# bdsaglam/torch-scae

Measured on AMD Instinct MI355X. Metric: images/sec SCAE fwd+bwd, MNIST 40x40 bs=128, 1/2/4/8 MI355X, higher is better.
Workload: dtype f32

## Files before the change

### torch_scae_amd/csrc/conv_resident.hip

```cpp
#include <cstdlib>

#include "bf16x6.h"
#include "mfma_pipe.h"
#include "conv_first_dev.h"

namespace {
namespace pipe = scae_pipe;
using scae_first::ConvGeom;
constexpr int NT = 256;

struct ResArgs {
  const float *in, *wp, *bias, *post_bias;
  float *out, *out_post;
  ConvGeom g;
  int G;
};

template <int MI>
__global__ __launch_bounds__(NT, 2) void conv_res_fwd_kernel(ResArgs a) {
  constexpr bool X6 = true;
  extern __shared__ __attribute__((aligned(1024))) float smem[];
  const int tid = threadIdx.x, wid = __builtin_amdgcn_readfirstlane(tid >> 6), lane = tid & 63,
            li = lane & 31, lk = lane >> 5;
  const ConvGeom &g = a.g;
  const int ntiles = g.Cout / 32;
  const int nt = blockIdx.x % ntiles, img0 = (blockIdx.x / ntiles) * a.G;
  const int nimg = min(a.G, g.B - img0);
  const int ipix = g.IH * g.IW, opix = g.OH * g.OW;
  const int SP = g.Cin / 4;
  {
    const pipe::rsrc_t rin =
        pipe::make_rsrc(a.in, (unsigned)((size_t)g.B * ipix * g.Cin * 4));
    const int units = a.G * ipix * SP, pieces = (units + 63) / 64;
    const int valid = nimg * ipix;
    for (int j = wid; j < pieces; j += 4) {
      const int u = j * 64 + lane, p = u / SP, s = u - p * SP;
      const int vo = p < valid ? (((img0 * ipix + p) * g.Cin) + ((s ^ (p & 15)) << 2)) * 4
                               : pipe::DMA_ZERO;
      pipe::dma16(rin, smem + j * 256, vo, 0);
    }
  }
  const int rows = nimg * opix;
  int pbase[MI];
#pragma unroll
  for (int mi = 0; mi < MI; ++mi) {
    const int r = min(mi * 32 + li, rows - 1);
    const int n = r / opix, rem = r - n * opix, oh = rem / g.OW, ow = rem - oh * g.OW;
    pbase[mi] = n * ipix + oh * g.stride * g.IW + ow * g.stride;
  }
  const int CB = g.Cin / 32;
  const int CPT = CB / 4;
  const int NCW = 9 * CPT;
  const uint4 *wq = reinterpret_cast<const uint4 *>(a.wp) + (size_t)nt * (9 * CB) * 384 + lane;
  constexpr int NS = !X6 ? 1 : (MI == 1 ? 3 : 1);
  pipe::f32x16 acc[MI], accl[X6 ? MI : 1][NS];
#pragma unroll
  for (int mi = 0; mi < MI; ++mi)
#pragma unroll
    for (int e = 0; e < 16; ++e) {
      acc[mi][e] = 0.f;
      if (X6) {
#pragma unroll
        for (int n = 0; n < NS; ++n) accl[mi][n][e] = 0.f;
      }
    }
  uint4 bq[2][2][3];
  auto load_b = [&](int c, int buf) {
    const int tap = c / CPT, cb = wid + 4 * (c - tap * CPT);
    const uint4 *src = wq + (size_t)(tap * CB + cb) * 384;
#pragma unroll
    for (int qp = 0; qp < 2; ++qp)
#pragma unroll
      for (int pl = 0; pl < 3; ++pl) bq[buf][qp][pl] = src[(qp * 3 + pl) * 64];
  };
  load_b(0, 0);
  pipe::wait_vm<0>();
  __syncthreads();
  auto chunk = [&](int c, int buf) {
    if (c + 1 < NCW) load_b(c + 1, buf ^ 1);
    const int tap = c / CPT, cb = wid + 4 * (c - tap * CPT);
    const int kh = tap / 3, kw = tap - 3 * kh;
    const int slot0 = cb * 8 + lk * 4;
    const float *ap[MI];
    int sw[MI];
#pragma unroll
    for (int mi = 0; mi < MI; ++mi) {
      const int p = pbase[mi] + kh * g.IW + kw;
      ap[mi] = smem + p * g.Cin;
      sw[mi] = p & 15;
    }
    if (X6) {
#pragma unroll
      for (int qp = 0; qp < 2; ++qp) {
        scae_x6::Split3 bs;
        bs.hi = __builtin_bit_cast(scae_x6::bf16x8, bq[buf][qp][0]);
        bs.mid = __builtin_bit_cast(scae_x6::bf16x8, bq[buf][qp][1]);
        bs.lo = __builtin_bit_cast(scae_x6::bf16x8, bq[buf][qp][2]);
        scae_x6::Split3 as[MI];
#pragma unroll
        for (int mi = 0; mi < MI; ++mi) {
          const float4 a0 = pipe::lds4(ap[mi] + (((slot0 + 2 * qp) ^ sw[mi]) << 2));
          const float4 a1 = pipe::lds4(ap[mi] + (((slot0 + 2 * qp + 1) ^ sw[mi]) << 2));
          as[mi] = scae_x6::split3(a0, a1);
        }
#define SCAE_X6_STEP(AP, BP, N)                                                                   \
  _Pragma("unroll") for (int mi = 0; mi < MI; ++mi) accl[mi][(N) % NS] =                          \
      __builtin_amdgcn_mfma_f32_32x32x16_bf16(as[mi].AP, bs.BP, accl[mi][(N) % NS], 0, 0, 0);
        SCAE_X6_STEP(hi, lo, 0)
        SCAE_X6_STEP(lo, hi, 1)
        SCAE_X6_STEP(mid, mid, 2)
        SCAE_X6_STEP(hi, mid, 0)
        SCAE_X6_STEP(mid, hi, 1)
#undef SCAE_X6_STEP
#pragma unroll
        for (int mi = 0; mi < MI; ++mi)
          acc[mi] = __builtin_amdgcn_mfma_f32_32x32x16_bf16(as[mi].hi, bs.hi, acc[mi], 0, 0, 0);
      }
    }
  };
  for (int c = 0; c < NCW; c += 2) {
    chunk(c, 0);
    if (c + 1 < NCW) chunk(c + 1, 1);
  }
  if (X6) {
#pragma unroll
    for (int mi = 0; mi < MI; ++mi) {
      pipe::f32x16 small = accl[mi][0];
#pragma unroll
      for (int n = 1; n < NS; ++n) small += accl[mi][n];
      acc[mi] += small;
    }
  }
  __syncthreads();
#pragma unroll
  for (int mi = 0; mi < MI; ++mi)
#pragma unroll
    for (int e = 0; e < 16; ++e) smem[((wid * MI + mi) * 16 + e) * 64 + lane] = acc[mi][e];
  const int col = nt * 32 + li;
  const float bn = a.bias[col];
  float pb[MI][4];
  const int row0 = 8 * wid + 4 * lk;
  if (a.out_post) {
#pragma unroll
    for (int mi = 0; mi < MI; ++mi)
#pragma unroll
      for (int e = 0; e < 4; ++e) {
        const int r = min(mi * 32 + row0 + e, rows - 1);
        pb[mi][e] = a.post_bias[(size_t)col * opix + r % opix];
      }
  }
  __syncthreads();
  const unsigned obytes = (unsigned)((size_t)g.B * opix * g.Cout * 4);
  const pipe::rsrc_t ro = pipe::make_rsrc(a.out, obytes);
  const pipe::rsrc_t rp = pipe::make_rsrc(a.out_post ? a.out_post : a.out, obytes);
#pragma unroll
  for (int mi = 0; mi < MI; ++mi)
#pragma unroll
    for (int e = 0; e < 4; ++e) {
      float v = 0.f;
#pragma unroll
      for (int w = 0; w < 4; ++w) v += smem[((w * MI + mi) * 16 + 4 * wid + e) * 64 + lane];
      const int r = mi * 32 + row0 + e;
      const float o = fmaxf(v + bn, 0.f);
      const int off = r < rows ? ((img0 * opix + r) * g.Cout + col) * 4 : pipe::DMA_ZERO;
      __builtin_amdgcn_raw_buffer_store_b32(__builtin_bit_cast(int, o), ro, off, 0, 0);
      if (a.out_post)
        __builtin_amdgcn_raw_buffer_store_b32(__builtin_bit_cast(int, o + pb[mi][e]), rp, off, 0, 0);
    }
}

struct ResPlan {
  int G, MI;
  size_t lds;
};
bool res_plan(const ConvGeom &g, ResPlan &p, int force_g) {
  if (g.stride < 1 || g.stride > 2 || g.Cin % 128 || g.Cout % 32) return false;
  const int opix = g.OH * g.OW, ipix = g.IH * g.IW;
  double best = 0.;
  p.G = 0;
  for (int G = 1; G <= 8 && G <= g.B; ++G) {
    if (force_g > 0 && G != force_g) continue;
    const int MI = (G * opix + 31) / 32;
    const size_t stage = ((size_t)G * ipix * g.Cin * 4 + 1023) & ~(size_t)1023;
    const size_t lds = std::max(stage, (size_t)4 * MI * 16 * 64 * 4);
    if (MI > 4 || lds > (force_g > 0 ? 150 : 64) * 1024) break;
    const double use = (double)G * opix / (32. * MI);
    if (use > best + 1e-9) best = use, p.G = G, p.MI = MI, p.lds = lds;
  }
  return p.G > 0;
}
}

extern "C" int scae_conv3x3_fwd_res_supported(int B, int IH, int IW, int Cin, int Cout, int stride) {
  if (B <= 0 || IH < 3 || IW < 3 || Cin <= 0 || Cout <= 0 || stride <= 0) return 0;
  ConvGeom g{B, IH, IW, (IH - 3) / stride + 1, (IW - 3) / stride + 1, Cin, Cout, stride};
  ResPlan p;
  return res_plan(g, p, 0) ? 1 : 0;
}

extern "C" int scae_conv3x3_fwd_res_f32(const float *in, const float *wp, const float *bias,
                                        float *out, const float *post_bias, float *out_post, int B,
                                        int IH, int IW, int Cin, int Cout, int stride, int group,
                                        void *stream) {
  SCAE_REQUIRE(in && wp && bias && out && (!out_post || post_bias) && B > 0 && IH >= 3 && IW >= 3 &&
               Cin > 0 && Cout > 0 && stride > 0 && group >= 0);
  ConvGeom g{B, IH, IW, (IH - 3) / stride + 1, (IW - 3) / stride + 1, Cin, Cout, stride};
  ResPlan p;
  if (!res_plan(g, p, group)) return SCAE_ERR_UNSUPPORTED;
  ResArgs a{in, wp, bias, post_bias, out, out_post, g, p.G};
  const dim3 grid((Cout / 32) * ((B + p.G - 1) / p.G));
  hipStream_t st = (hipStream_t)stream;
#define SCAE_RES(M)                                                                              \
  case M: {                                                                                      \
    if (p.lds > 48 * 1024) {                                                                     \
      hipError_t e = hipFuncSetAttribute(reinterpret_cast<const void *>(conv_res_fwd_kernel<M>), \
                                         hipFuncAttributeMaxDynamicSharedMemorySize, (int)p.lds); \
      if (e != hipSuccess) return (int)e;                                                        \
    }                                                                                            \
    scae::launch(conv_res_fwd_kernel<M>, grid, dim3(NT), p.lds, st, a);                          \
    break;                                                                                       \
  }
  switch (p.MI) {
    SCAE_RES(1) SCAE_RES(2) SCAE_RES(3) SCAE_RES(4)
    default: return SCAE_ERR_UNSUPPORTED;
  }
#undef SCAE_RES
  return scae_launch_status();
}
```

Baseline: 269,500.

## Pre-split staged conv input into bf16x3 in LDS and share across two N tiles

The resident 3x3 conv kernel now splits each fp32 input into hi/mid/lo bf16 parts once, while staging it into LDS, using a 48-byte unit layout with an output-pixel-keyed swizzle. Before, every wave re-split the same activations for every tap and column tile. Blocks can also run 512 threads covering two 32-column output tiles, so one staged image is reused by twice as many columns. The LDS budget rises to 80KB and staging now goes through registers instead of direct DMA. In exchange, the small float-based division and the halved occupancy bound for NJ=2 could reduce latency hiding.

Result: faster. 273,600, median of 6 (+1.5%).

```diff
diff --git a/torch_scae_amd/csrc/conv_resident.hip b/torch_scae_amd/csrc/conv_resident.hip
--- a/torch_scae_amd/csrc/conv_resident.hip
+++ b/torch_scae_amd/csrc/conv_resident.hip
@@ -16,120 +16,149 @@
   int G;
 };
 
-template <int MI>
-__global__ __launch_bounds__(NT, 2) void conv_res_fwd_kernel(ResArgs a) {
-  constexpr bool X6 = true;
+constexpr int SU = 6;
+constexpr int UNIT_BYTES = 48;
+
+__device__ __forceinline__ int small_div(int p, float rd) { return (int)(((float)p + 0.5f) * rd); }
+
+template <int MI, int NJ>
+__global__ __launch_bounds__(NT * NJ, 2 / NJ) void conv_res_fwd_kernel(ResArgs a) {
+  constexpr int NTH = NT * NJ;
   extern __shared__ __attribute__((aligned(1024))) float smem[];
+  char *const simg = reinterpret_cast<char *>(smem);
   const int tid = threadIdx.x, wid = __builtin_amdgcn_readfirstlane(tid >> 6), lane = tid & 63,
             li = lane & 31, lk = lane >> 5;
   const ConvGeom &g = a.g;
-  const int ntiles = g.Cout / 32;
-  const int nt = blockIdx.x % ntiles, img0 = (blockIdx.x / ntiles) * a.G;
+  const int kp = wid & 3, nj = wid >> 2;
+  const int ntiles = g.Cout / (32 * NJ);
+  const int nt = (blockIdx.x % ntiles) * NJ + nj, img0 = (blockIdx.x / ntiles) * a.G;
   const int nimg = min(a.G, g.B - img0);
   const int ipix = g.IH * g.IW, opix = g.OH * g.OW;
-  const int SP = g.Cin / 4;
+  const int UP = g.Cin / 8;
+  const int rowb = UP * UNIT_BYTES;
+  const int sh = g.stride - 1;
+  const int CB = g.Cin / 32;
+  const int CPT = CB / 4;
+  const int NCW = 9 * CPT;
+  const uint4 *wq = reinterpret_cast<const uint4 *>(a.wp) + (size_t)nt * (9 * CB) * 384 + lane;
+  uint4 bq[2][2][3];
+  auto load_b = [&](int c, int buf) {
+    const int tap = c / CPT, cb = kp + 4 * (c - tap * CPT);
+    const uint4 *src = wq + (size_t)(tap * CB + cb) * 384;
+#pragma unroll
+    for (int qp = 0; qp < 2; ++qp)
+#pragma unroll
+      for (int pl = 0; pl < 3; ++pl) bq[buf][qp][pl] = src[(qp * 3 + pl) * 64];
+  };
+  load_b(0, 0);
   {
     const pipe::rsrc_t rin =
         pipe::make_rsrc(a.in, (unsigned)((size_t)g.B * ipix * g.Cin * 4));
-    const int units = a.G * ipix * SP, pieces = (units + 63) / 64;
-    const int valid = nimg * ipix;
-    for (int j = wid; j < pieces; j += 4) {
-      const int u = j * 64 + lane, p = u / SP, s = u - p * SP;
-      const int vo = p < valid ? (((img0 * ipix + p) * g.Cin) + ((s ^ (p & 15)) << 2)) * 4
-                               : pipe::DMA_ZERO;
-      pipe::dma16(rin, smem + j * 256, vo, 0);
+    const int units = a.G * ipix * UP, valid = nimg * ipix;
+    const float ripix = 1.f / (float)ipix, riw = 1.f / (float)g.IW;
+    const int dp = NTH / UP, ds = NTH - dp * UP;
+    int p = tid / UP, s = tid - p * UP;
+    for (int ub = 0; ub < units; ub += SU * NTH) {
+      const int u0 = ub + tid;
+      scae_x6::u32x4 v[SU][2];
+      int dst[SU];
+#pragma unroll
+      for (int k = 0; k < SU; ++k) {
+        if (ub + k * NTH >= units) break;
+        const bool in = u0 + k * NTH < units;
+        const int vo = in && p < valid ? ((img0 * ipix + p) * g.Cin + s * 8) * 4 : pipe::DMA_ZERO;
+        v[k][0] = __builtin_amdgcn_raw_buffer_load_b128(rin, vo, 0, 0);
+        v[k][1] = __builtin_amdgcn_raw_buffer_load_b128(rin, vo, 16, 0);
+        const int n = small_div(p, ripix), rem = p - n * ipix;
+        const int ih = small_div(rem, riw), iw = rem - ih * g.IW;
+        const int key = n * opix + (ih >> sh) * g.OW + (iw >> sh);
+        dst[k] = in ? p * rowb + (s ^ (key & 15)) * UNIT_BYTES : units * UNIT_BYTES;
+        s += ds, p += dp;
+        if (s >= UP) s -= UP, ++p;
+      }
+#pragma unroll
+      for (int k = 0; k < SU; ++k) {
+        if (ub + k * NTH >= units) break;
+        const scae_x6::Split3 sp = scae_x6::split3(__builtin_bit_cast(float4, v[k][0]),
+                                                   __builtin_bit_cast(float4, v[k][1]));
+        uint4 *d = reinterpret_cast<uint4 *>(simg + dst[k]);
+        d[0] = __builtin_bit_cast(uint4, sp.hi);
+        d[1] = __builtin_bit_cast(uint4, sp.mid);
+        d[2] = __builtin_bit_cast(uint4, sp.lo);
+      }
     }
   }
   const int rows = nimg * opix;
-  int pbase[MI];
+  int pbase[MI], kbase[MI];
 #pragma unroll
   for (int mi = 0; mi < MI; ++mi) {
     const int r = min(mi * 32 + li, rows - 1);
     const int n = r / opix, rem = r - n * opix, oh = rem / g.OW, ow = rem - oh * g.OW;
     pbase[mi] = n * ipix + oh * g.stride * g.IW + ow * g.stride;
-  }
-  const int CB = g.Cin / 32;
-  const int CPT = CB / 4;
-  const int NCW = 9 * CPT;
-  const uint4 *wq = reinterpret_cast<const uint4 *>(a.wp) + (size_t)nt * (9 * CB) * 384 + lane;
-  constexpr int NS = !X6 ? 1 : (MI == 1 ? 3 : 1);
-  pipe::f32x16 acc[MI], accl[X6 ? MI : 1][NS];
+    kbase[mi] = r;
+  }
+  constexpr int NS = MI == 1 ? 3 : 1;
+  pipe::f32x16 acc[MI], accl[MI][NS];
 #pragma unroll
   for (int mi = 0; mi < MI; ++mi)
 #pragma unroll
     for (int e = 0; e < 16; ++e) {
       acc[mi][e] = 0.f;
-      if (X6) {
-#pragma unroll
-        for (int n = 0; n < NS; ++n) accl[mi][n][e] = 0.f;
-      }
-    }
-  uint4 bq[2][2][3];
-  auto load_b = [&](int c, int buf) {
-    const int tap = c / CPT, cb = wid + 4 * (c - tap * CPT);
-    const uint4 *src = wq + (size_t)(tap * CB + cb) * 384;
-#pragma unroll
-    for (int qp = 0; qp < 2; ++qp)
-#pragma unroll
-      for (int pl = 0; pl < 3; ++pl) bq[buf][qp][pl] = src[(qp * 3 + pl) * 64];
-  };
-  load_b(0, 0);
-  pipe::wait_vm<0>();
+#pragma unroll
+      for (int n = 0; n < NS; ++n) accl[mi][n][e] = 0.f;
+    }
   __syncthreads();
   auto chunk = [&](int c, int buf) {
     if (c + 1 < NCW) load_b(c + 1, buf ^ 1);
-    const int tap = c / CPT, cb = wid + 4 * (c - tap * CPT);
+    const int tap = c / CPT, cb = kp + 4 * (c - tap * CPT);
     const int kh = tap / 3, kw = tap - 3 * kh;
-    const int slot0 = cb * 8 + lk * 4;
-    const float *ap[MI];
+    const int unit0 = cb * 4 + lk * 2;
+    const char *ap[MI];
     int sw[MI];
 #pragma unroll
     for (int mi = 0; mi < MI; ++mi) {
-      const int p = pbase[mi] + kh * g.IW + kw;
-      ap[mi] = smem + p * g.Cin;
-      sw[mi] = p & 15;
-    }
-    if (X6) {
-#pragma unroll
-      for (int qp = 0; qp < 2; ++qp) {
-        scae_x6::Split3 bs;
-        bs.hi = __builtin_bit_cast(scae_x6::bf16x8, bq[buf][qp][0]);
-        bs.mid = __builtin_bit_cast(scae_x6::bf16x8, bq[buf][qp][1]);
-        bs.lo = __builtin_bit_cast(scae_x6::bf16x8, bq[buf][qp][2]);
-        scae_x6::Split3 as[MI];
-#pragma unroll
-        for (int mi = 0; mi < MI; ++mi) {
-          const float4 a0 = pipe::lds4(ap[mi] + (((slot0 + 2 * qp) ^ sw[mi]) << 2));
-          const float4 a1 = pipe::lds4(ap[mi] + (((slot0 + 2 * qp + 1) ^ sw[mi]) << 2));
-          as[mi] = scae_x6::split3(a0, a1);
-        }
+      ap[mi] = simg + (pbase[mi] + kh * g.IW + kw) * rowb;
+      sw[mi] = (kbase[mi] + (kh >> sh) * g.OW + (kw >> sh)) & 15;
+    }
+#pragma unroll
+    for (int qp = 0; qp < 2; ++qp) {
+      scae_x6::Split3 bs;
+      bs.hi = __builtin_bit_cast(scae_x6::bf16x8, bq[buf][qp][0]);
+      bs.mid = __builtin_bit_cast(scae_x6::bf16x8, bq[buf][qp][1]);
+      bs.lo = __builtin_bit_cast(scae_x6::bf16x8, bq[buf][qp][2]);
+      scae_x6::Split3 as[MI];
+#pragma unroll
+      for (int mi = 0; mi < MI; ++mi) {
+        const uint4 *src =
+            reinterpret_cast<const uint4 *>(ap[mi] + ((unit0 + qp) ^ sw[mi]) * UNIT_BYTES);
+        as[mi].hi = __builtin_bit_cast(scae_x6::bf16x8, src[0]);
+        as[mi].mid = __builtin_bit_cast(scae_x6::bf16x8, src[1]);
+        as[mi].lo = __builtin_bit_cast(scae_x6::bf16x8, src[2]);
+      }
 #define SCAE_X6_STEP(AP, BP, N)                                                                   \
   _Pragma("unroll") for (int mi = 0; mi < MI; ++mi) accl[mi][(N) % NS] =                          \
       __builtin_amdgcn_mfma_f32_32x32x16_bf16(as[mi].AP, bs.BP, accl[mi][(N) % NS], 0, 0, 0);
-        SCAE_X6_STEP(hi, lo, 0)
-        SCAE_X6_STEP(lo, hi, 1)
-        SCAE_X6_STEP(mid, mid, 2)
-        SCAE_X6_STEP(hi, mid, 0)
-        SCAE_X6_STEP(mid, hi, 1)
+      SCAE_X6_STEP(hi, lo, 0)
+      SCAE_X6_STEP(lo, hi, 1)
+      SCAE_X6_STEP(mid, mid, 2)
+      SCAE_X6_STEP(hi, mid, 0)
+      SCAE_X6_STEP(mid, hi, 1)
 #undef SCAE_X6_STEP
 #pragma unroll
-        for (int mi = 0; mi < MI; ++mi)
-          acc[mi] = __builtin_amdgcn_mfma_f32_32x32x16_bf16(as[mi].hi, bs.hi, acc[mi], 0, 0, 0);
-      }
+      for (int mi = 0; mi < MI; ++mi)
+        acc[mi] = __builtin_amdgcn_mfma_f32_32x32x16_bf16(as[mi].hi, bs.hi, acc[mi], 0, 0, 0);
     }
   };
   for (int c = 0; c < NCW; c += 2) {
     chunk(c, 0);
     if (c + 1 < NCW) chunk(c + 1, 1);
   }
-  if (X6) {
-#pragma unroll
-    for (int mi = 0; mi < MI; ++mi) {
-      pipe::f32x16 small = accl[mi][0];
-#pragma unroll
-      for (int n = 1; n < NS; ++n) small += accl[mi][n];
-      acc[mi] += small;
-    }
+#pragma unroll
+  for (int mi = 0; mi < MI; ++mi) {
+    pipe::f32x16 small = accl[mi][0];
+#pragma unroll
+    for (int n = 1; n < NS; ++n) small += accl[mi][n];
+    acc[mi] += small;
   }
   __syncthreads();
 #pragma unroll
@@ -139,7 +168,7 @@
   const int col = nt * 32 + li;
   const float bn = a.bias[col];
   float pb[MI][4];
-  const int row0 = 8 * wid + 4 * lk;
+  const int row0 = 8 * kp + 4 * lk;
   if (a.out_post) {
 #pragma unroll
     for (int mi = 0; mi < MI; ++mi)
@@ -159,7 +188,8 @@
     for (int e = 0; e < 4; ++e) {
       float v = 0.f;
 #pragma unroll
-      for (int w = 0; w < 4; ++w) v += smem[((w * MI + mi) * 16 + 4 * wid + e) * 64 + lane];
+      for (int w = 0; w < 4; ++w)
+        v += smem[(((nj * 4 + w) * MI + mi) * 16 + 4 * kp + e) * 64 + lane];
       const int r = mi * 32 + row0 + e;
       const float o = fmaxf(v + bn, 0.f);
       const int off = r < rows ? ((img0 * opix + r) * g.Cout + col) * 4 : pipe::DMA_ZERO;
@@ -170,7 +200,7 @@
 }
 
 struct ResPlan {
-  int G, MI;
+  int G, MI, NJ;
   size_t lds;
 };
 bool res_plan(const ConvGeom &g, ResPlan &p, int force_g) {
@@ -181,11 +211,12 @@
   for (int G = 1; G <= 8 && G <= g.B; ++G) {
     if (force_g > 0 && G != force_g) continue;
     const int MI = (G * opix + 31) / 32;
-    const size_t stage = ((size_t)G * ipix * g.Cin * 4 + 1023) & ~(size_t)1023;
-    const size_t lds = std::max(stage, (size_t)4 * MI * 16 * 64 * 4);
-    if (MI > 4 || lds > (force_g > 0 ? 150 : 64) * 1024) break;
+    const size_t stage = ((size_t)G * ipix * (g.Cin / 8) + 1) * UNIT_BYTES;
+    const int NJ = g.Cout % 64 == 0 && MI <= 2 ? 2 : 1;
+    const size_t lds = std::max(stage, (size_t)4 * NJ * MI * 16 * 64 * 4);
+    if (MI > 4 || lds > (force_g > 0 ? 150 : 80) * 1024) break;
     const double use = (double)G * opix / (32. * MI);
-    if (use > best + 1e-9) best = use, p.G = G, p.MI = MI, p.lds = lds;
+    if (use > best + 1e-9) best = use, p.G = G, p.MI = MI, p.NJ = NJ, p.lds = lds;
   }
   return p.G > 0;
 }
@@ -208,20 +239,21 @@
   ResPlan p;
   if (!res_plan(g, p, group)) return SCAE_ERR_UNSUPPORTED;
   ResArgs a{in, wp, bias, post_bias, out, out_post, g, p.G};
-  const dim3 grid((Cout / 32) * ((B + p.G - 1) / p.G));
+  const dim3 grid((Cout / (32 * p.NJ)) * ((B + p.G - 1) / p.G));
   hipStream_t st = (hipStream_t)stream;
-#define SCAE_RES(M)                                                                              \
-  case M: {                                                                                      \
+#define SCAE_RES(M, J)                                                                           \
+  case M * 2 + J - 1: {                                                                          \
     if (p.lds > 48 * 1024) {                                                                     \
-      hipError_t e = hipFuncSetAttribute(reinterpret_cast<const void *>(conv_res_fwd_kernel<M>), \
-                                         hipFuncAttributeMaxDynamicSharedMemorySize, (int)p.lds); \
+      hipError_t e =                                                                             \
+          hipFuncSetAttribute(reinterpret_cast<const void *>(conv_res_fwd_kernel<M, J>),         \
+                              hipFuncAttributeMaxDynamicSharedMemorySize, (int)p.lds);           \
       if (e != hipSuccess) return (int)e;                                                        \
     }                                                                                            \
-    scae::launch(conv_res_fwd_kernel<M>, grid, dim3(NT), p.lds, st, a);                          \
+    scae::launch(conv_res_fwd_kernel<M, J>, grid, dim3(NT * J), p.lds, st, a);                   \
     break;                                                                                       \
   }
-  switch (p.MI) {
-    SCAE_RES(1) SCAE_RES(2) SCAE_RES(3) SCAE_RES(4)
+  switch (p.MI * 2 + p.NJ - 1) {
+    SCAE_RES(1, 1) SCAE_RES(2, 1) SCAE_RES(3, 1) SCAE_RES(4, 1) SCAE_RES(1, 2) SCAE_RES(2, 2)
     default: return SCAE_ERR_UNSUPPORTED;
   }
 #undef SCAE_RES
```
